# cvlab-kaist/CoPoNeRF

Hardware: AMD Instinct MI355X
Metric: rendered rays/sec (RealEstate10K-shaped 256x256 stereo pair, full-image render, 64 samples/ray) (higher is better)
Workload: dtype f16 (fp16-input/fp32-accumulate MFMA for the per-sample MLPs; f32 decoder; f64 geometry island); 1 GPU; configs[1]: 256x256 stereo pair (narrow rig), full-image render 65536 rays x 64 samples, 1 pair(s) per GPU, render path only (z/rel_pose/flow given, val=True); chunk_rays=65536, lanes=1, pairs_per_gpu=1

## Files before the change

### coponerf_amd/_hip.py

```python
from __future__ import annotations

import ctypes
import os
import re
from typing import Dict, List

_HERE = os.path.dirname(os.path.abspath(__file__))
LIB_PATH = os.environ.get("COPONERF_HIP_LIB") or os.path.join(_HERE, "libcoponerf_hip.so")
HEADER_PATH = os.path.join(os.path.dirname(_HERE), "include", "coponerf_hip.h")

_P, _I, _F = ctypes.c_void_p, ctypes.c_int, ctypes.c_float

SIGNATURES: Dict[str, List] = {
    "cpn_stream_create_cu_range": [_I, _I, ctypes.POINTER(ctypes.c_void_p)],
    "cpn_stream_destroy": [_P],
    "cpn_project_rays": [_P, _P, ctypes.c_longlong, _I, _I, _I, _P, _P, _P, _P],
    "cpn_sample_geometry": [_P, _P, _P, _P, _I, _I, _I, _I, _I, _I, _P, _P, _P, _P, _P, _P, _P],
    "cpn_nchw_to_nhwc_f16": [_P, _P, _I, _I, _I, _I, _P],
    "cpn_pack_weight_f16": [_P, _I, _I, _P, _I, _P],
    "cpn_pack_encode_weights": [_P, _I, _P, _P, _P],
    "cpn_node_features": [_P, _P, _P, _I, _I, _I, _P, _P],
    "cpn_encode_key": [_P, _P, _I, _I, _P, _P, _P, _P, _P, _P, _P, _I, _I, _I, _I, _I, _I, _P, _P, _I, _P],
    "cpn_local_units": [_I, _P, _P, _P, _I, _P, _P, _P, _I, _P, _P, _I, _P, _P, _I, _P, _P, _I, _I, _I, _I, _I, _I, _P, _P, _P, _P],
    "cpn_attend_units": [_I, _P, _P, _P, _I, _P, _P, _P, _I, _P, _P, _I, _P, _P, _I, _P, _P, _P, _I, _I, _I, _I, _I, _I, _P, _P, _P, _P, _P],
    "cpn_local_hidden": [_P, _P, _P, _I, _P, _P, _I, _I, _I, _I, _I, _I, _P, _P],
    "cpn_gemm_f16": [_P, _I, _P, _I, _P, _P, _I, _I, _I, _I, _I, _I, _P],
    "cpn_pack_gemm_frags": [_P, _I, _I, _I, _P, _P],
    "cpn_gemm_f16_fewrows": [_P, _I, _P, _P, _P, _I, _I, _I, _I, _I, _P],
    "cpn_attend_hidden": [_P, _P, _P, _P, _I, _I, _I, _I, _I, _I, _P, _P, _P],
    "cpn_node_features_f32": [_P, _P, _P, _I, _I, _I, _P, _P],
    "cpn_encode_hidden_f32": [_P, _P, _I, _I, _P, _P, _P, _P, _I, _I, _I, _I, _I, _I, _P, _P],
    "cpn_attend_hidden_f32": [_P, _P, _P, _I, _I, _I, _I, _I, _I, _P, _P, _P],
    "cpn_logit_guard": [_P, _I, _I, _I, _I, _I, _I, _P, _I, _P],
    "cpn_select_rays": [_P, _I, _F, _P, _P, _P],
    "cpn_encode_hidden_f32_rays": [_P, _P, _I, _I, _P, _P, _P, _P, _I, _I, _I, _I, _P, _I, _I, _P, _P],
    "cpn_attend_hidden_f32_rays": [_P, _P, _P, _I, _I, _I, _I, _P, _I, _I, _P, _P, _P],
    "cpn_linear_f32": [_P, _I, _P, _I, _P, _P, _I, _P, _I, _I, _I, _I, _I, _I, _P],
    "cpn_lightfield_decode": [_P, _P, _P, _P, _I, _I, _I, _P, _P, _P, _P],
    "cpn_ray_outputs": [_P, _P, _P, ctypes.c_longlong, _P, _P, _P, _I, _I, _I, _I, _P, _P, _P, _P, _P, _P, _P, _P],
    "cpn_attend_hidden_bwd": [_P, _P, _P, _P, _P, _P, _I, _I, _I, _I, _I, _I, _P, _P, _P, _P, _P],
    "cpn_attend_hidden_bwd_f32": [_P, _P, _P, _P, _P, _P, _I, _I, _I, _I, _I, _I, _P, _P, _P, _P],
    "cpn_hid_grad_combine": [_P, _P, _P, _P, _P, _P, _I, _I, _I, _I, _I, _I, _P, _P],
    "cpn_gemm_f16_combine": [_P, _I, _P, _I, _P, _P, _P, _P, _P, _I, _I, _I, _I, _I, _I, _I, _P, _P],
    "cpn_gemm_f16_combine_hs": [_P, _I, _P, _I, _P, _P, _P, _P, _P, _I, _I, _I, _I, _I, _I, _I, _P, _P],
    "cpn_gemm_f16_masked": [_P, _I, _P, _I, _P, _I, _P, _I, _I, _I, _I, _P],
    "cpn_wgrad_skinny_f16": [_P, _P, _I, ctypes.c_longlong, _P, _P, _P],
    "cpn_wgrad_tall_f16": [_P, _I, _P, _I, ctypes.c_longlong, _I, _I, _P, _P, _P, _P],
    "cpn_local_hidden_bwd": [_P, _P, _P, _P, _P, _I, _I, _I, _I, _P, _P, _P, _P],
    "cpn_gather_rows_bwd_level3": [_P, _I, _I, _I, _I, _P, _P, _I, _I, _I, _I, _I, _I, _P, _P, _P],
    "cpn_scatter_rows_tables": [_P, _I, _I, _I, _P, _P, _I, _I, _I, _I, _I, _I, _P, _P, _P],
    "cpn_node_features_bwd": [_P, _I, _I, _I, _P, _P, _P, _P],
    "cpn_scale_to_f16": [_P, ctypes.c_longlong, _F, _P, _P, _P, _P],
# ... 151 lines not shown
```

### coponerf_amd/csrc/attend_units.hip

```cpp
#include <algorithm>

#include "hid_sum.h"
#include "local_units_body.h"

namespace {

constexpr int HC = 1664;
constexpr int NCHUNK = HC / 8;
constexpr int NL = 4;
constexpr int NS = 2 * TG;
constexpr int AU_THREADS = (NL + NS) * 64;
constexpr int RU = HID_BLOCK_ROWS;
constexpr int LDS_MAX = 160 * 1024;

__device__ __forceinline__ float wave_max(float v) {
#pragma unroll
    for (int o = 32; o > 0; o >>= 1) v = fmaxf(v, __shfl_xor(v, o));
    return v;
}
__device__ __forceinline__ float wave_sum(float v) {
#pragma unroll
    for (int o = 32; o > 0; o >>= 1) v += __shfl_xor(v, o);
    return v;
}
// ... 76 lines not shown
        int b, r;
        size_t lray;
        const __half* hp;
    };
    auto ray_of = [&](unsigned k) {
        Ray o;
        const long long gq = geo.group0 + bid + (long long)k * nwg;
        o.b = (int)(gq / geo.groups_per_b);
        o.r = (int)(gq % geo.groups_per_b) * TG + j;
        const long long rayrel = (long long)o.b * R + o.r - geo.ray0;
        o.live = k < nmy && o.r < R && rayrel >= 0 && rayrel < geo.nrays;
        o.lray = (size_t)max(0LL, min(rayrel, (long long)geo.nrays - 1));
        o.hp = hid + o.lray * T * HC;
        return o;
    };
    auto issue = [&](const Ray& ray, half8 (&h0)[RU], half8 (&h1)[RU], int row) {
#pragma unroll
        for (int u = 0; u < RU; ++u) {
            const __half* rp = ray.hp + (size_t)(row + u) * HC;
            h0[u] = __builtin_nontemporal_load(reinterpret_cast<const half8*>(rp + off0));
            h1[u] = __builtin_nontemporal_load(reinterpret_cast<const half8*>(rp + off1));
        }
    };
    auto pin = [] {
        asm volatile("" ::: "memory");
        __builtin_amdgcn_sched_barrier(0);
    };
    half8 a0[RU], a1[RU], b0[RU], b1[RU];
    Ray nxt = ray_of(0);
    if (nxt.live && npair > 0) issue(nxt, a0, a1, 0);
    for (unsigned k = 0; k < nmy; ++k) {
        const Ray ray = nxt;
        nxt = ray_of(k + 1);
        const bool pre = nxt.live && npair > 0;
        const int b = ray.b, r = ray.r;
        group_barrier();
        if (!ray.live) {
            if (pre) issue(nxt, a0, a1, 0);
            continue;
        }

        const float* lg = ring + (k & 1) * (TG * T) + j * T;
        float* wt = wbuf + j * T;
        float lmax = -INFINITY;
        for (int row = lane; row < T; row += 64) lmax = fmaxf(lmax, lg[row] / 11.31f);
        const float gmax = wave_max(lmax);
        float ps[4] = {0.f, 0.f, 0.f, 0.f};
        for (int base = 0; base < T; base += 256) {
#pragma unroll
            for (int q = 0; q < 4; ++q) {
                const int row = base + q * 64 + lane;
                if (row < T) ps[q] += __expf(lg[row] / 11.31f - gmax);
            }
        }
#pragma unroll
        for (int q = 0; q < 4; ++q) ps[q] = wave_sum(ps[q]);
        const float inv = 1.0f / ((ps[0] + ps[1]) + (ps[2] + ps[3]));
        for (int row = lane; row < T; row += 64) {
            const float w = __expf(lg[row] / 11.31f - gmax) * inv;
            wt[row] = w;
            if (at_wt && half == 0) {
                const int v = row / S, s = row - v * S;
                at_wt[(((size_t)(b * V + v)) * R + r) * S + s] = w;
            }
        }
        asm volatile("s_waitcnt lgkmcnt(0)" ::: "memory");

        float acc0[8] = {0, 0, 0, 0, 0, 0, 0, 0}, acc1[8] = {0, 0, 0, 0, 0, 0, 0, 0};
        auto consume = [&](const half8 (&h0)[RU], const half8 (&h1)[RU], int row) {
#pragma unroll
            for (int u = 0; u < RU; ++u) {
                const float w = wt[row + u];
                hid_row_acc<true>(acc0, w, h0[u]);
                hid_row_acc<true>(acc1, w, h1[u]);
            }
        };
        if (npair > 0) {
            for (int p = 0; p + 1 < npair; ++p) {
                issue(ray, b0, b1, (2 * p + 1) * RU);
                pin();
                consume(a0, a1, 2 * p * RU);
                pin();
                issue(ray, a0, a1, (2 * p + 2) * RU);
                pin();
                consume(b0, b1, (2 * p + 1) * RU);
                pin();
            }
            issue(ray, b0, b1, (2 * npair - 1) * RU);
            pin();
            consume(a0, a1, (2 * npair - 2) * RU);
            pin();
            if (pre) issue(nxt, a0, a1, 0);
            pin();
            consume(b0, b1, (2 * npair - 1) * RU);
            pin();
        }
        for (int row = npair * 2 * RU; row < T; ++row) {
            const half8 h0 = __builtin_nontemporal_load(reinterpret_cast<const half8*>(ray.hp + (size_t)row * HC + off0));
            const half8 h1 = __builtin_nontemporal_load(reinterpret_cast<const half8*>(ray.hp + (size_t)row * HC + off1));
            const float w = wt[row];
            if (row < T - T % HID_BLOCK_ROWS) {
                hid_row_acc<true>(acc0, w, h0);
                hid_row_acc<true>(acc1, w, h1);
            } else {
                hid_row_acc<false>(acc0, w, h0);
                hid_row_acc<false>(acc1, w, h1);
            }
        }
        half8 o0, o1;
#pragma unroll
        for (int e = 0; e < 8; ++e) {
            o0[e] = (_Float16)acc0[e];
            o1[e] = (_Float16)acc1[e];
        }
        *reinterpret_cast<half8*>(hbar + ray.lray * HC + c0 * 8) = o0;
        if (live1) *reinterpret_cast<half8*>(hbar + ray.lray * HC + c1 * 8) = o1;
    }
}

template <int MODE>
int launch(const UnitArgs& args, const UnitGeo& geo, const __half* hid, __half* hbar, float* at_wt, float* logits, hipStream_t stream) {
    const int T = geo.V * geo.S;
    const size_t lds = unit_lds_bytes<MODE>() + (size_t)3 * TG * T * sizeof(float);
    CPN_REQUIRE(lds <= (size_t)LDS_MAX, CPN_E_SHAPE,
                "cpn_attend_units: V*S = %d needs %zu B of LDS (weights + 3 x 4 rays of logits / weights), the CU has %d", T, lds, LDS_MAX);
    auto kern = attend_units_kernel<MODE>;
    static bool attr_set = false;
    if (!attr_set) {
        hipError_t e = hipFuncSetAttribute((const void*)kern, hipFuncAttributeMaxDynamicSharedMemorySize, LDS_MAX);
        if (e != hipSuccess) {
            cpn_set_error("cpn_attend_units: cannot reserve %d B of LDS: %s", LDS_MAX, hipGetErrorString(e));
// ... 38 lines not shown
```

### coponerf_amd/csrc/gemm_f16.hip

```cpp
#include <algorithm>

#include "common.h"

namespace {

constexpr int BM = 256;
constexpr int BK = 64;
constexpr int ROW_BYTES = BK * 2;

typedef __attribute__((address_space(3))) void lds_void;
typedef const __attribute__((address_space(1))) void glb_void;

template <int NT>
struct Cfg {
    static constexpr int BN = NT * 16;
    static constexpr int UNITS_A = BM / 8;
    static constexpr int UNITS_B = BN / 8;
    static constexpr int UNITS = UNITS_A + UNITS_B;
    static constexpr int A_BYTES = BM * ROW_BYTES;
    static constexpr int B_BYTES = BN * ROW_BYTES;
    static constexpr int A_SLOTS = 3;
    static constexpr int B_SLOTS = 2;
    static constexpr int DUMP_BYTES = (UNITS_B % 8) ? 8 * 1024 : 0;
    static constexpr int LDS_BYTES = A_SLOTS * A_BYTES + B_SLOTS * B_BYTES + DUMP_BYTES;
// ... 7 lines not shown
    const int xcd = b & 7, idx = b >> 3;
    const int wg_x = (nwg >> 3) + (xcd < (nwg & 7) ? 1 : 0);
    const int q = total >> 3, r = total & 7;
    TileWalk t;
    t.begin = xcd < r ? xcd * (q + 1) : r * (q + 1) + (xcd - r) * q;
    t.end = t.begin + q + (xcd < r ? 1 : 0);
    t.step = wg_x;
    t.cur = t.begin + idx;
    return t;
}

struct CombineArgs {
    const float* w1; const float* dh1; const float* w2; const float* dh2;
    int V, R, S, ray0;
    int accum;
};
#ifndef CPN_HID_READ_NT
#define CPN_HID_READ_NT 1
#endif
template <int NT, bool OUT_F32, bool RELU, int DOT = 0>
__global__ __launch_bounds__(512) void gemm_f16_kernel(const __half* __restrict__ A, int lda,
                                                             const __half* __restrict__ W, int ldw,
                                                             const float* __restrict__ bias,
                                                             void* __restrict__ Cv, int ldc, int M, int K32, int n_tiles,
                                                             int total_tiles, const __half* __restrict__ Q = nullptr,
                                                             int ldq = 0, const __half* __restrict__ W2 = nullptr,
                                                             int ldw2 = 0, const float* __restrict__ bias2 = nullptr,
                                                             CombineArgs ca = CombineArgs{}) {
    using C_ = Cfg<NT>;
    constexpr int A_AUX = 0;
// ... 282 lines not shown
                    }
                }
                __builtin_amdgcn_fence(__ATOMIC_RELEASE, "wavefront");
            }
        } else {
#pragma unroll
            for (int nt = 0; nt < NT; ++nt) {
                const int n = n0 + nt * 16 + (lane >> 4) * 4;
                const f32x4 bv = *reinterpret_cast<const f32x4*>(bias + n);
#pragma unroll
                for (int mt = 0; mt < 2; ++mt) {
                    const int m = m0 + wave * 32 + mt * 16 + (lane & 15);
                    if (m >= M) continue;
                    f32x4 v = acc[mt][nt] + bv;
                    if (ca.accum) v += *reinterpret_cast<const f32x4*>((const float*)Cv + (size_t)m * ldc + n);
                    if (RELU) {
#pragma unroll
                        for (int i = 0; i < 4; ++i) v[i] = fmaxf(v[i], 0.0f);
                    }
                    *reinterpret_cast<f32x4*>((float*)Cv + (size_t)m * ldc + n) = v;
                }
            }
        }
    }
#undef CPN_INTERLEAVE_READS_MFMA
}

template <int NT, bool OUT_F32, bool RELU>
int launch(const __half* A, int lda, const __half* W, int ldw, const float* bias, void* C, int ldc, int M, int N,
           int K32, hipStream_t stream, int accum = 0) {
    using C_ = Cfg<NT>;
    const size_t lds = C_::LDS_BYTES;
    auto kern = gemm_f16_kernel<NT, OUT_F32, RELU>;
    static bool attr_set = false;
    if (!attr_set) {
        hipError_t e = hipFuncSetAttribute((const void*)kern, hipFuncAttributeMaxDynamicSharedMemorySize, (int)lds);
        if (e != hipSuccess) {
            cpn_set_error("cpn_gemm_f16: cannot reserve %zu B of LDS: %s", lds, hipGetErrorString(e));
            return (int)e;
        }
        attr_set = true;
    }
    const int n_tiles = N / C_::BN;
    const long long total = (long long)cpn_cdiv(M, BM) * n_tiles;
    if (total >= (1LL << 31)) {
        cpn_set_error("cpn_gemm_f16: %lld output tiles exceed the 32-bit tile index", total);
        return CPN_E_SHAPE;
    }
    const int num_cu = cpn_stream_cus((void*)stream);
    dim3 grid((unsigned)std::min<long long>(total, num_cu));
    hipLaunchKernelGGL(kern, grid, dim3(512), lds, stream, A, lda, W, ldw, bias, C, ldc, M, K32, n_tiles, (int)total,
                       (const __half*)nullptr, 0, (const __half*)nullptr, 0, (const float*)nullptr,
                       CombineArgs{nullptr, nullptr, nullptr, nullptr, 0, 0, 0, 0, accum});
    CPN_LAUNCH_CHECK("cpn_gemm_f16");
    return 0;
}

template <int NT>
int launch_combine(const __half* A, int lda, const __half* W, int ldw, const __half* hid, int ldh, const CombineArgs& ca,
                   __half* out, int ld, int M, int N, int K32, hipStream_t stream) {
    using C_ = Cfg<NT>;
    const size_t lds = C_::LDS_BYTES;
    auto kern = gemm_f16_kernel<NT, false, false, 3>;
    static bool attr_set = false;
    if (!attr_set) {
        hipError_t e = hipFuncSetAttribute((const void*)kern, hipFuncAttributeMaxDynamicSharedMemorySize, (int)lds);
        if (e != hipSuccess) {
            cpn_set_error("cpn_gemm_f16_combine: cannot reserve %zu B of LDS: %s", lds, hipGetErrorString(e));
// ... 36 lines not shown
    out[i] = *reinterpret_cast<const half8*>(W + (size_t)(t * 16 + (lane & 15)) * ldw + ks * 32 + (lane >> 4) * 8);
}

#ifndef CPN_FEW_NT
#define CPN_FEW_NT 4
#endif
#ifndef CPN_FEW_DEPTH
#define CPN_FEW_DEPTH 4
#endif
#ifndef CPN_FEW_RT
#define CPN_FEW_RT 2
#endif
constexpr int FEW_NT = CPN_FEW_NT, FEW_RT = CPN_FEW_RT;
__global__ __launch_bounds__(256) void gemm_f16_fewrows_kernel(const __half* __restrict__ A, int lda,
                                                               const half8* __restrict__ Wp, const float* __restrict__ bias,
                                                               float* __restrict__ C, int ldc, int M, int N, int K32, int relu) {
    constexpr int NT = FEW_NT, RT = FEW_RT, D = CPN_FEW_DEPTH;
    const int lane = threadIdx.x & 63, wave = threadIdx.x >> 6;
    const int r = lane & 15, g = lane >> 4;
    const int m0 = blockIdx.x * 16 * RT;
    const int ntiles = N >> 4;
    const int tile0 = (blockIdx.y * 4 + wave) * NT;
    if (tile0 >= ntiles) return;
    const int rl = lane >> 2, pl = lane & 3;
    const int to_frag = (4 * r + g) * 4;
    const __half* ap[RT];
#pragma unroll
    for (int q = 0; q < RT; ++q) {
        const int row = m0 + q * 16 + rl < M ? m0 + q * 16 + rl : M - 1;
        ap[q] = A + (size_t)row * lda + pl * 8;
    }
// ... 68 lines not shown
        for (int q = 0; q < RT; ++q) xl[q] = frag(xl[q]);
#pragma unroll
        for (int t = 0; t < NT; ++t)
#pragma unroll
            for (int q = 0; q < RT; ++q) acc[q][t] = __builtin_amdgcn_mfma_f32_16x16x32_f16(wl[t], xl[q], acc[q][t], 0, 0, 0);
    }
#pragma unroll
    for (int q = 0; q < RT; ++q) {
        const int m = m0 + q * 16 + r;
        if (m >= M) continue;
#pragma unroll
        for (int t = 0; t < NT; ++t) {
            if (tile0 + t >= ntiles) continue;
            const int n = (tile0 + t) * 16 + g * 4;
            f32x4 v = acc[q][t] + *reinterpret_cast<const f32x4*>(bias + n);
            if (relu) {
#pragma unroll
                for (int i = 0; i < 4; ++i) v[i] = fmaxf(v[i], 0.0f);
            }
            *reinterpret_cast<f32x4*>(C + (size_t)m * ldc + n) = v;
        }
    }
}

}

extern "C" int cpn_pack_gemm_frags(const uint16_t* W, int ldw, int N, int K, uint16_t* out, void* stream) {
    CPN_REQUIRE(W && out, CPN_E_ARG, "cpn_pack_gemm_frags: null pointer");
    CPN_REQUIRE(N > 0 && (N % 16) == 0 && K > 0 && (K % 32) == 0 && ldw >= K && (ldw % 8) == 0, CPN_E_SHAPE,
                "cpn_pack_gemm_frags: need N %% 16 == 0, K %% 32 == 0, ldw >= K (got N=%d K=%d ldw=%d)", N, K, ldw);
// ... 3 lines not shown
                       K / 32, (half8*)out);
    CPN_LAUNCH_CHECK("cpn_pack_gemm_frags");
    return 0;
}

extern "C" int cpn_gemm_f16_fewrows(const uint16_t* A, int lda, const uint16_t* Wp, const float* bias, float* C, int ldc, int M,
                                    int N, int K, int relu, void* stream) {
    CPN_REQUIRE(A && Wp && bias && C, CPN_E_ARG, "cpn_gemm_f16_fewrows: null pointer");
    CPN_REQUIRE(M > 0 && N > 0 && (N % 16) == 0 && K > 0 && (K % 32) == 0, CPN_E_SHAPE,
                "cpn_gemm_f16_fewrows: need N %% 16 == 0 and K %% 32 == 0 (got N=%d K=%d)", N, K);
    CPN_REQUIRE(lda >= K && (lda % 8) == 0 && ldc >= N && (ldc % 4) == 0, CPN_E_SHAPE, "cpn_gemm_f16_fewrows: bad leading dimension");
    CPN_REQUIRE(((uintptr_t)A % 16) == 0 && ((uintptr_t)Wp % 16) == 0 && ((uintptr_t)C % 16) == 0 && ((uintptr_t)bias % 16) == 0,
                CPN_E_ARG, "cpn_gemm_f16_fewrows: pointers must be 16-byte aligned");
    dim3 grid(cpn_cdiv(M, 16 * FEW_RT), cpn_cdiv(N / 16, 4 * FEW_NT));
    hipLaunchKernelGGL(gemm_f16_fewrows_kernel, grid, dim3(256), 0, (hipStream_t)stream, (const __half*)A, lda, (const half8*)Wp, bias,
                       C, ldc, M, N, K / 32, relu);
    CPN_LAUNCH_CHECK("cpn_gemm_f16_fewrows");
    return 0;
}

extern "C" int cpn_gemm_f16(const uint16_t* A, int lda, const uint16_t* W, int ldw, const float* bias, void* C,
                            int ldc, int M, int N, int K, int relu, int out_f32, void* stream) {
    CPN_REQUIRE(A && W && bias && C, CPN_E_ARG, "cpn_gemm_f16: null pointer");
    CPN_REQUIRE(M > 0 && N > 0 && K > 0 && (K % 32) == 0, CPN_E_SHAPE, "cpn_gemm_f16: K=%d must be a multiple of 32", K);
    CPN_REQUIRE(lda >= K && ldw >= K && (lda % 8) == 0 && (ldw % 8) == 0, CPN_E_SHAPE,
                "cpn_gemm_f16: lda=%d / ldw=%d must be >= K=%d and multiples of 8 halves", lda, ldw, K);
    CPN_REQUIRE((long long)256 * lda * 2 < (1LL << 31) && (long long)N * ldw * 2 < (1LL << 31), CPN_E_SHAPE,
                "cpn_gemm_f16: tile exceeds the 32-bit buffer offset range");
    CPN_REQUIRE(ldc >= N && (ldc % 8) == 0, CPN_E_SHAPE, "cpn_gemm_f16: ldc=%d must be >= N and a multiple of 8", ldc);
    CPN_REQUIRE(((uintptr_t)A % 16) == 0 && ((uintptr_t)W % 16) == 0 && ((uintptr_t)C % 16) == 0 &&
                    ((uintptr_t)bias % 16) == 0, CPN_E_ARG, "cpn_gemm_f16: pointers must be 16-byte aligned");
    const hipStream_t s = (hipStream_t)stream;
    const __half* a = (const __half*)A;
    const __half* w = (const __half*)W;
    if (N % 208 == 0) return dispatch<13>(a, lda, w, ldw, bias, C, ldc, M, N, K / 32, relu, out_f32, s);
    if (N % 128 == 0) return dispatch<8>(a, lda, w, ldw, bias, C, ldc, M, N, K / 32, relu, out_f32, s);
    cpn_set_error("cpn_gemm_f16: N=%d is neither a multiple of 208 nor of 128", N);
    return CPN_E_SHAPE;
}

namespace {

template <int LDH>
int gemm_f16_combine(const char* name, const uint16_t* dkh, int lda, const uint16_t* Wt, int ldw, const uint16_t* hid,
                     const float* w1, const float* dh1, const float* w2, const float* dh2, int B, int V, int R, int S, int ray0,
                     int nrays, int K, uint16_t* out, void* stream) {
    CPN_REQUIRE(dkh && Wt && hid && out && (!w1 || dh1) && (!w2 || dh2), CPN_E_ARG, "%s: null pointer", name);
    CPN_REQUIRE(B > 0 && V == 2 && R > 0 && S > 0 && (S % 16) == 0, CPN_E_SHAPE, "%s: need V == 2, S %% 16 == 0", name);
    CPN_REQUIRE(ray0 >= 0 && nrays > 0 && (long long)ray0 + nrays <= (long long)B * R, CPN_E_SHAPE,
                "%s: ray range outside B*R", name);
    CPN_REQUIRE(K > 0 && (K % 32) == 0 && lda >= K && ldw >= K && (lda % 8) == 0 && (ldw % 8) == 0, CPN_E_SHAPE,
                "%s: bad K / leading dimension", name);
// ... 49 lines not shown
```

### coponerf_amd/csrc/linear_f32.hip

```cpp
#include "common.h"

namespace {

#ifndef CPN_LIN_DEPTH
#define CPN_LIN_DEPTH 2
#endif
template <int NT>
__global__ __launch_bounds__(256) void linear_f32_kernel(const float* __restrict__ X, int ldx,
                                                         const float* __restrict__ W, int ldw,
                                                         const float* __restrict__ bias,
                                                         const float* __restrict__ res, int ldr,
                                                         float* __restrict__ Y, int ldy, int M, int N, int K,
                                                         int relu_in, int relu_out) {
    constexpr int D = CPN_LIN_DEPTH;
    const int lane = threadIdx.x & 63, wave = threadIdx.x >> 6;
    const int m0 = (blockIdx.x * 4 + wave) * 16;
    const int t0 = blockIdx.y * NT;
    if (m0 >= M) return;
    const int fi = lane & 15, fg = lane >> 4;
    int xr = m0 + fi;
    xr = xr < M ? xr : M - 1;
    const float* xp = X + (size_t)xr * ldx + fg * 4;
    f32x4 acc[NT];
#pragma unroll
// ... 57 lines not shown
            continue;
        }
#pragma unroll
        for (int i = 0; i < 4; ++i) {
            const int n = n0 + i;
            if (n >= N) continue;
            float v = acc[t][i];
            if (bias) v += bias[n];
            if (res) v += res[(size_t)m * ldr + n];
            if (relu_out) v = fmaxf(v, 0.0f);
            Y[(size_t)m * ldy + n] = v;
        }
    }
}

}

extern "C" int cpn_linear_f32(const float* X, int ldx, const float* W, int ldw, const float* bias, const float* res,
                              int ldr, float* Y, int ldy, int M, int N, int K, int relu_in, int relu_out,
                              void* stream) {
    CPN_REQUIRE(X && W && Y, CPN_E_ARG, "cpn_linear_f32: null pointer");
    CPN_REQUIRE(M > 0 && N > 0 && N <= 128 && K > 0 && (K % 16) == 0, CPN_E_SHAPE,
                "cpn_linear_f32: need N<=128 and K%%16==0 (got N=%d K=%d)", N, K);
    CPN_REQUIRE(ldx >= K && ldw >= K && (ldx % 4) == 0 && (ldw % 4) == 0 && ldy >= N && (!res || ldr >= N),
                CPN_E_SHAPE, "cpn_linear_f32: bad leading dimensions");
    CPN_REQUIRE(((uintptr_t)X % 16) == 0 && ((uintptr_t)W % 16) == 0, CPN_E_ARG, "cpn_linear_f32: X/W must be 16-B aligned");
    const hipStream_t s = (hipStream_t)stream;
    dim3 grid(cpn_cdiv(M, 64)), block(256);
    const int ntiles = (int)cpn_cdiv(N, 16);
    if (N <= 16)
// ... 13 lines not shown
```

### coponerf_amd/render.py

```python
from __future__ import annotations

import ctypes
import math
import os
from typing import Dict, List, Optional, Sequence, Tuple

import torch

from . import _hip, render_f32
from ._hip import call

V = 2


def _ptr(t: Optional[torch.Tensor]) -> int:
    return 0 if t is None else t.data_ptr()


def _stream() -> int:
    return _hip.stream_handle()


def _flat_on_device(mats: Sequence[Optional[torch.Tensor]]) -> Optional[torch.Tensor]:
    live = [m for m in mats if m is not None]
# ... 271 lines not shown
            return func(*args, **kwargs)


class RenderEngine:

    GEMM_WEIGHTS = {
        "key_map_2": (128, 128, 128),
        "query_embed_2": (128, 128, 128),
        "query_repeat_embed_2": (128, 128, 128),
    }

    WORKSPACE_SHARE = 0.25
    FREE_SHARE = 0.5
    MAX_AUTO_CHUNK = 65536
    ATTEND_UNITS_MAX_T = 1684
    FEW_ROWS = 4096
    AUTO_THRESHOLD = 0.5062
    PRECISIONS = ("f16", "f32", "auto")
    TRAIN_PRECISIONS = ("f16", "f32")
    SETTINGS = ("chunk_rays", "lanes", "grad_scale_target", "call_lanes", "lazy_pixel_val", "precision", "f32_chunk_rays",
                "auto_threshold", "train_precision")

    def __init__(self, chunk_rays: int = 0, lanes: int = 1):
        self.chunk_rays = int(chunk_rays) or int(os.environ.get("COPONERF_CHUNK_RAYS", "0"))
        self.grad_scale_target = 256.0
        self.lanes = max(1, int(lanes))
        self._lane_streams: List[torch.cuda.Stream] = []
        self.precision = os.environ.get("COPONERF_PRECISION", "f16")
        self.f32_chunk_rays = 16384
        self.auto_threshold = self.AUTO_THRESHOLD
# ... 550 lines not shown
        score = self._buf("guard.score", (nray_total,), f32, dev) if auto else None
        C = min(self.chunk_rays if self.chunk_rays > 0 else self._auto_chunk(S, dev, nray_total), nray_total)
        T = V * S
        fused = T <= self.ATTEND_UNITS_MAX_T
        nchunks = (nray_total + C - 1) // C
        nlanes = min(self.lanes, nchunks)
        if nlanes > 1 and (len(self._lane_streams) < nlanes or self._lane_streams[0].device != dev):
            self._lane_streams = [torch.cuda.Stream(device=dev) for _ in range(nlanes)]
        main = torch.cuda.current_stream()

        def lane_buffers(lane):
            t = lambda name, shape, dt: self._buf(f"{name}.{lane}", shape, dt, dev)
            rows128 = ((C + 3) // 4 + B + 1) * V * ((S + 3) // 4) * 16
            return {"lg": t("lg", (C * T,), f32) if (auto or not fused) else None,
                    "z1": t("z1", (C, 416), f32), "ze": t("ze", (C, 128), f32), "addq": t("addq", (C, 128), f32),
                    "hbar": t("hbar", (C, 1664), f16), "zs": t("zs", (C, 416), f32),
                    "hid": t("hid", (C * T * 2, 832), f16), "khf": t("khf", (rows128, 128), f16)}

        def timed(name, flops, fn):
            prof = self.profile
            if prof is None:
                return fn()
            e0, e1 = torch.cuda.Event(enable_timing=True), torch.cuda.Event(enable_timing=True)
            e0.record()
            fn()
            e1.record()
            prof.setdefault(name, []).append((e0, e1, flops))

        def value_fold(s, hbar, out, m):
            if m <= self.FEW_ROWS:
                fn = lambda: call("cpn_gemm_f16_fewrows", hbar.data_ptr(), 1664, w["value_fold.wpk"].data_ptr(),
                                  w["value_fold.b"].data_ptr(), out.data_ptr(), 416, m, 416, 1664, 0, s)
            else:
                fn = lambda: call("cpn_gemm_f16", hbar.data_ptr(), 1664, w["value_fold.w16"].data_ptr(), 1664,
                                  w["value_fold.b"].data_ptr(), out.data_ptr(), 416, m, 416, 1664, 0, 1, s)
            timed("gemm_f16:value_fold", 2.0 * m * 416 * 1664, fn)

        def run_chunk(ray0, bf, s):
            n = min(C, nray_total - ray0)
            rows2 = n * T * 2
            timed("encode_key", 2.0 * rows2 * 832 * 835, lambda: call(
                "cpn_encode_key", tabs[0].data_ptr(), maps[3].data_ptr(), H, W, pixel_val.data_ptr(), sec_grid.data_ptr(),
                pe6.data_ptr(), w["enc.frag"].data_ptr(), w["query_encode_latent.b"].data_ptr(), w["key_fold.wpk"].data_ptr(),
                w["key_fold.b"].data_ptr(), B, V, R, S, ray0, n, bf["hid"].data_ptr(), bf["khf"].data_ptr(), 1, s))
            lg = bf["lg"].data_ptr() if (auto or not fused) else 0
            r1 = (0, loc8.data_ptr(), coords9.data_ptr(), w["query_embed.w"].data_ptr(), 16,
                  w["query_embed.b"].data_ptr(), 0, w["query_embed_2.w16"].data_ptr(), 128, w["query_embed_2.b"].data_ptr(),
                  w["key_map_2.w16"].data_ptr(), 128, w["key_map_2.b"].data_ptr(), 0, 0, 0, bf["khf"].data_ptr())
            if fused:
                timed("attend_units:round1", 2.0 * n * T * (128 * (128 + 128 + 16) + 1664), lambda: call(
                    "cpn_attend_units", *r1, bf["hid"].data_ptr(), B, V, R, S, ray0, n, lvu.data_ptr(),
                    bf["hbar"].data_ptr(), at_wt.data_ptr(), lg, s))
            else:
                timed("local_units:query_embed+key_map_2", 2.0 * n * T * 128 * (128 + 128 + 16), lambda: call(
                    "cpn_local_units", *r1, B, V, R, S, ray0, n, 0, lvu.data_ptr(), lg, s))
                timed("attend_hidden:round1", 2.0 * n * T * 1664, lambda: call(
                    "cpn_attend_hidden", 0, 0, lg, bf["hid"].data_ptr(), B, V, R, S, ray0, n,
                    bf["hbar"].data_ptr(), at_wt.data_ptr(), s))
            if auto:
                timed("logit_guard:round1", 0.0, lambda: call(
                    "cpn_logit_guard", lg, B, V, R, S, ray0, n, score.data_ptr(), 0, s))
            z1, ze, addq = bf["z1"], bf["ze"], bf["addq"]
            value_fold(s, bf["hbar"], z1, n)
            call("cpn_linear_f32", z1.data_ptr(), 416, w["encode_latent.w"].data_ptr(), 416,
                 w["encode_latent.b"].data_ptr(), 0, 0, ze.data_ptr(), 128, n, 128, 416, 0, 0, s)
            call("cpn_linear_f32", ze.data_ptr(), 128, w["query_repeat_embed.w_z"].data_ptr(), 128, 0, 0, 0,
                 addq.data_ptr(), 128, n, 128, 128, 0, 0, s)
            r2 = (2, loc8.data_ptr(), coords9.data_ptr(), w["query_repeat_embed.w_l"].data_ptr(), 16,
                  w["query_repeat_embed.b"].data_ptr(), addq.data_ptr(), w["query_repeat_embed_2.w16"].data_ptr(), 128,
                  w["query_repeat_embed_2.b"].data_ptr(), w["query_embed_2.w16"].data_ptr(), 128, w["query_embed_2.b"].data_ptr(),
                  w["query_embed.w"].data_ptr(), 16, w["query_embed.b"].data_ptr(), 0)
            if fused:
                timed("attend_units:round2", 2.0 * n * T * (128 * (2 * 128 + 2 * 16) + 1664), lambda: call(
                    "cpn_attend_units", *r2, bf["hid"].data_ptr(), B, V, R, S, ray0, n, lvu.data_ptr(),
                    bf["hbar"].data_ptr(), 0, lg, s))
            else:
                timed("local_units:round2+query_embed", 2.0 * n * T * 128 * (2 * 128 + 2 * 16), lambda: call(
                    "cpn_local_units", *r2, B, V, R, S, ray0, n, 0, lvu.data_ptr(), lg, s))
                timed("attend_hidden:round2", 2.0 * n * T * 1664, lambda: call(
                    "cpn_attend_hidden", 0, 0, lg, bf["hid"].data_ptr(), B, V, R, S, ray0, n,
                    bf["hbar"].data_ptr(), 0, s))
            if auto:
                timed("logit_guard:round2", 0.0, lambda: call(
                    "cpn_logit_guard", lg, B, V, R, S, ray0, n, score.data_ptr(), 1, s))
            value_fold(s, bf["hbar"], bf["zs"], n)
            torch.add(bf["zs"][:n], z1[:n], alpha=float(V), out=zl[ray0:ray0 + n])

        dims = (B, R, S, H, W)
        f32_inputs = lambda: self._f32_inputs(pre[8], w, H, W)
        if self.precision == "f32":
            render_f32.per_sample(*f32_inputs(), g, zl, at_wt, dims, self.f32_chunk_rays, self._buf, s)
        elif nlanes == 1:
            bf = lane_buffers(0)
            for ray0 in range(0, nray_total, C):
                run_chunk(ray0, bf, s)
        else:
            ready = torch.cuda.Event()
            ready.record()
            for ci, ray0 in enumerate(range(0, nray_total, C)):
                lane = ci % nlanes
                st = self._lane_streams[lane]
# ... 43 lines not shown
```

### include/coponerf_hip.h

```cpp
#ifndef COPONERF_HIP_H
#define COPONERF_HIP_H

#include <stdint.h>

#ifdef __cplusplus
extern "C" {
#endif

#define CPN_ABI_VERSION 12

#define CPN_E_ARG   (-1)
#define CPN_E_SHAPE (-2)

#define CPN_CAM_STRIDE 96
#define CPN_CAM_TQ    0
#define CPN_CAM_M     16
#define CPN_CAM_AOWN  32
#define CPN_CAM_AOTH  48
#define CPN_CAM_KQ    64
#define CPN_CAM_KC    68
#define CPN_CAM_KO    72
#define CPN_CAM_KN    76


// ... 28 lines not shown
int cpn_encode_key(const uint16_t* tab, const uint16_t* map3, int H, int W, const float* pixel_val,
                   const float* sec_grid, const float* pe6, const uint16_t* wfrag, const float* bias,
                   const uint16_t* kwring, const float* kbias, int B, int V, int R, int S, int ray0, int nrays,
                   uint16_t* hid, uint16_t* kh, int kh_units, void* stream);
long long cpn_encode_units(int B, int R, int S, int ray0, int nrays);
int cpn_local_units(int mode, const float* loc8, const float* coords9, const float* w1, int ldw1, const float* b1,
                    const float* add, const uint16_t* w2, int ldw2, const float* b2, const uint16_t* wk2, int ldwk2,
                    const float* bk2, const float* w1b, int ldw1b, const float* b1b, const uint16_t* kh_u, int B, int V,
                    int R, int S, int ray0, int nrays, uint16_t* ce_u, const float* lv_u, float* logits, void* stream);

int cpn_gemm_f16(const uint16_t* A, int lda, const uint16_t* W, int ldw, const float* bias,
                 void* C, int ldc, int M, int N, int K, int relu, int out_f32, void* stream);
int cpn_pack_gemm_frags(const uint16_t* W, int ldw, int N, int K, uint16_t* out, void* stream);
int cpn_gemm_f16_fewrows(const uint16_t* A, int lda, const uint16_t* Wp, const float* bias, float* C, int ldc, int M, int N,
                         int K, int relu, void* stream);

int cpn_attend_hidden(const uint16_t* qa, const uint16_t* qb, const float* logits, const uint16_t* hid, int B, int V,
                      int R, int S, int ray0, int nrays, uint16_t* hbar, float* at_wt, void* stream);

int cpn_attend_units(int mode, const float* loc8, const float* coords9, const float* w1, int ldw1, const float* b1,
                     const float* add, const uint16_t* w2, int ldw2, const float* b2, const uint16_t* wk2, int ldwk2,
                     const float* bk2, const float* w1b, int ldw1b, const float* b1b, const uint16_t* kh_u, const uint16_t* hid,
                     int B, int V, int R, int S, int ray0, int nrays, const float* lv_u, uint16_t* hbar, float* at_wt,
                     float* logits, void* stream);

int cpn_linear_f32(const float* X, int ldx, const float* W, int ldw, const float* bias, const float* res, int ldr,
                   float* Y, int ldy, int M, int N, int K, int relu_in, int relu_out, void* stream);

#define CPN_LIGHTFIELD_PACK_FLOATS (128 * 32 + 128 + 3 * (128 * 416 + 128 + 2 * (128 * 128 + 128)) + 16 * 128 + 16)
int cpn_lightfield_decode(const float* coords9, const float* z_local, const float* wpack, const uint8_t* overlaps,
                          int B, int V, int R, float* rgb, float* valid, float* rgb_raw, void* stream);

#define CPN_RAYC_STRIDE 64
int cpn_ray_outputs(const float* at_wt, const float* pt, const float* uv, long long uv_batch_stride, const float* rayc,
                    const uint8_t* mask2, const float* flow_up, int B, int V, int R, int S, long long* at_wt_max,
                    float* depth_ray, float* t_to_c1, float* t_to_c2, uint8_t* mask_c2, uint8_t* match_mask,
                    float* c2_to_c1, void* stream);


int cpn_node_features_f32(const float* map0, const float* map1, const float* map2, int H, int W, int nimg, float* feat,
                          void* stream);

// ... 180 lines not shown
```

Before: 2.936 million rays/s.

## Fuse residual add into value_fold GEMM and chain two f32 linears

```diff
diff --git a/coponerf_amd/_hip.py b/coponerf_amd/_hip.py
--- a/coponerf_amd/_hip.py
+++ b/coponerf_amd/_hip.py
@@ -27,6 +27,8 @@
     "cpn_gemm_f16": [_P, _I, _P, _I, _P, _P, _I, _I, _I, _I, _I, _I, _P],
     "cpn_pack_gemm_frags": [_P, _I, _I, _I, _P, _P],
     "cpn_gemm_f16_fewrows": [_P, _I, _P, _P, _P, _I, _I, _I, _I, _I, _P],
+    "cpn_gemm_f16_res": [_P, _I, _P, _I, _P, _P, _I, _F, _P, _I, _I, _I, _I, _P],
+    "cpn_gemm_f16_fewrows_res": [_P, _I, _P, _P, _P, _I, _F, _P, _I, _I, _I, _I, _P],
     "cpn_attend_hidden": [_P, _P, _P, _P, _I, _I, _I, _I, _I, _I, _P, _P, _P],
     "cpn_node_features_f32": [_P, _P, _P, _I, _I, _I, _P, _P],
     "cpn_encode_hidden_f32": [_P, _P, _I, _I, _P, _P, _P, _P, _I, _I, _I, _I, _I, _I, _P, _P],
@@ -36,6 +38,7 @@
     "cpn_encode_hidden_f32_rays": [_P, _P, _I, _I, _P, _P, _P, _P, _I, _I, _I, _I, _P, _I, _I, _P, _P],
     "cpn_attend_hidden_f32_rays": [_P, _P, _P, _I, _I, _I, _I, _P, _I, _I, _P, _P, _P],
     "cpn_linear_f32": [_P, _I, _P, _I, _P, _P, _I, _P, _I, _I, _I, _I, _I, _I, _P],
+    "cpn_linear2_f32": [_P, _I, _P, _I, _P, _P, _I, _P, _P, _I, _P, _I, _I, _I, _P],
     "cpn_lightfield_decode": [_P, _P, _P, _P, _I, _I, _I, _P, _P, _P, _P],
     "cpn_ray_outputs": [_P, _P, _P, ctypes.c_longlong, _P, _P, _P, _I, _I, _I, _I, _P, _P, _P, _P, _P, _P, _P, _P],
     "cpn_attend_hidden_bwd": [_P, _P, _P, _P, _P, _P, _I, _I, _I, _I, _I, _I, _P, _P, _P, _P, _P],
diff --git a/coponerf_amd/csrc/attend_units.hip b/coponerf_amd/csrc/attend_units.hip
--- a/coponerf_amd/csrc/attend_units.hip
+++ b/coponerf_amd/csrc/attend_units.hip
@@ -114,12 +114,15 @@
         o.hp = hid + o.lray * T * HC;
         return o;
     };
+    auto load_row = [&](const Ray& ray, unsigned voff, int row) {
+        const __amdgpu_buffer_rsrc_t rs = __builtin_amdgcn_make_buffer_rsrc((void*)ray.hp, 0, T * HC * 2, 0x00020000);
+        return __builtin_bit_cast(half8, __builtin_amdgcn_raw_buffer_load_b128(rs, (int)voff * 2, row * HC * 2, 2));
+    };
     auto issue = [&](const Ray& ray, half8 (&h0)[RU], half8 (&h1)[RU], int row) {
 #pragma unroll
         for (int u = 0; u < RU; ++u) {
-            const __half* rp = ray.hp + (size_t)(row + u) * HC;
-            h0[u] = __builtin_nontemporal_load(reinterpret_cast<const half8*>(rp + off0));
-            h1[u] = __builtin_nontemporal_load(reinterpret_cast<const half8*>(rp + off1));
+            h0[u] = load_row(ray, off0, row + u);
+            h1[u] = load_row(ray, off1, row + u);
         }
     };
     auto pin = [] {
@@ -128,17 +131,12 @@
     };
     half8 a0[RU], a1[RU], b0[RU], b1[RU];
     Ray nxt = ray_of(0);
-    if (nxt.live && npair > 0) issue(nxt, a0, a1, 0);
+    if (npair > 0) issue(nxt, a0, a1, 0);
     for (unsigned k = 0; k < nmy; ++k) {
         const Ray ray = nxt;
         nxt = ray_of(k + 1);
-        const bool pre = nxt.live && npair > 0;
         const int b = ray.b, r = ray.r;
         group_barrier();
-        if (!ray.live) {
-            if (pre) issue(nxt, a0, a1, 0);
-            continue;
-        }
 
         const float* lg = ring + (k & 1) * (TG * T) + j * T;
         float* wt = wbuf + j * T;
@@ -159,7 +157,7 @@
         for (int row = lane; row < T; row += 64) {
             const float w = __expf(lg[row] / 11.31f - gmax) * inv;
             wt[row] = w;
-            if (at_wt && half == 0) {
+            if (at_wt && half == 0 && ray.live) {
                 const int v = row / S, s = row - v * S;
                 at_wt[(((size_t)(b * V + v)) * R + r) * S + s] = w;
             }
@@ -174,30 +172,35 @@
                 hid_row_acc<true>(acc0, w, h0[u]);
                 hid_row_acc<true>(acc1, w, h1[u]);
             }
+        };
+        auto done = [&] {
+            asm volatile("" : "+v"(acc0[0]), "+v"(acc0[1]), "+v"(acc0[2]), "+v"(acc0[3]), "+v"(acc0[4]), "+v"(acc0[5]), "+v"(acc0[6]),
+                         "+v"(acc0[7]), "+v"(acc1[0]), "+v"(acc1[1]), "+v"(acc1[2]), "+v"(acc1[3]), "+v"(acc1[4]), "+v"(acc1[5]),
+                         "+v"(acc1[6]), "+v"(acc1[7])::"memory");
+            __builtin_amdgcn_sched_barrier(0);
         };
         if (npair > 0) {
             for (int p = 0; p + 1 < npair; ++p) {
                 issue(ray, b0, b1, (2 * p + 1) * RU);
                 pin();
                 consume(a0, a1, 2 * p * RU);
-                pin();
+                done();
                 issue(ray, a0, a1, (2 * p + 2) * RU);
                 pin();
                 consume(b0, b1, (2 * p + 1) * RU);
-                pin();
+                done();
             }
             issue(ray, b0, b1, (2 * npair - 1) * RU);
             pin();
             consume(a0, a1, (2 * npair - 2) * RU);
-            pin();
-            if (pre) issue(nxt, a0, a1, 0);
+            done();
+            issue(nxt, a0, a1, 0);
             pin();
             consume(b0, b1, (2 * npair - 1) * RU);
-            pin();
+            done();
         }
         for (int row = npair * 2 * RU; row < T; ++row) {
-            const half8 h0 = __builtin_nontemporal_load(reinterpret_cast<const half8*>(ray.hp + (size_t)row * HC + off0));
-            const half8 h1 = __builtin_nontemporal_load(reinterpret_cast<const half8*>(ray.hp + (size_t)row * HC + off1));
+            const half8 h0 = load_row(ray, off0, row), h1 = load_row(ray, off1, row);
             const float w = wt[row];
             if (row < T - T % HID_BLOCK_ROWS) {
                 hid_row_acc<true>(acc0, w, h0);
@@ -213,8 +216,8 @@
             o0[e] = (_Float16)acc0[e];
             o1[e] = (_Float16)acc1[e];
         }
-        *reinterpret_cast<half8*>(hbar + ray.lray * HC + c0 * 8) = o0;
-        if (live1) *reinterpret_cast<half8*>(hbar + ray.lray * HC + c1 * 8) = o1;
+        if (ray.live) *reinterpret_cast<half8*>(hbar + ray.lray * HC + c0 * 8) = o0;
+        if (ray.live && live1) *reinterpret_cast<half8*>(hbar + ray.lray * HC + c1 * 8) = o1;
     }
 }
 
diff --git a/coponerf_amd/csrc/gemm_f16.hip b/coponerf_amd/csrc/gemm_f16.hip
--- a/coponerf_amd/csrc/gemm_f16.hip
+++ b/coponerf_amd/csrc/gemm_f16.hip
@@ -45,6 +45,7 @@
     const float* w1; const float* dh1; const float* w2; const float* dh2;
     int V, R, S, ray0;
     int accum;
+    const float* res; int ldr; float alpha;
 };
 #ifndef CPN_HID_READ_NT
 #define CPN_HID_READ_NT 1
@@ -357,6 +358,11 @@
                     if (m >= M) continue;
                     f32x4 v = acc[mt][nt] + bv;
                     if (ca.accum) v += *reinterpret_cast<const f32x4*>((const float*)Cv + (size_t)m * ldc + n);
+                    if (ca.res) {
+                        const f32x4 z = *reinterpret_cast<const f32x4*>(ca.res + (size_t)m * ca.ldr + n);
+#pragma unroll
+                        for (int i = 0; i < 4; ++i) v[i] = __builtin_fmaf(ca.alpha, z[i], v[i]);
+                    }
                     if (RELU) {
 #pragma unroll
                         for (int i = 0; i < 4; ++i) v[i] = fmaxf(v[i], 0.0f);
@@ -371,7 +377,7 @@
 
 template <int NT, bool OUT_F32, bool RELU>
 int launch(const __half* A, int lda, const __half* W, int ldw, const float* bias, void* C, int ldc, int M, int N,
-           int K32, hipStream_t stream, int accum = 0) {
+           int K32, hipStream_t stream, int accum = 0, const float* res = nullptr, int ldr = 0, float alpha = 0.0f) {
     using C_ = Cfg<NT>;
     const size_t lds = C_::LDS_BYTES;
     auto kern = gemm_f16_kernel<NT, OUT_F32, RELU>;
@@ -394,7 +400,7 @@
     dim3 grid((unsigned)std::min<long long>(total, num_cu));
     hipLaunchKernelGGL(kern, grid, dim3(512), lds, stream, A, lda, W, ldw, bias, C, ldc, M, K32, n_tiles, (int)total,
                        (const __half*)nullptr, 0, (const __half*)nullptr, 0, (const float*)nullptr,
-                       CombineArgs{nullptr, nullptr, nullptr, nullptr, 0, 0, 0, 0, accum});
+                       CombineArgs{nullptr, nullptr, nullptr, nullptr, 0, 0, 0, 0, accum, res, ldr, alpha});
     CPN_LAUNCH_CHECK("cpn_gemm_f16");
     return 0;
 }
@@ -461,7 +467,8 @@
 constexpr int FEW_NT = CPN_FEW_NT, FEW_RT = CPN_FEW_RT;
 __global__ __launch_bounds__(256) void gemm_f16_fewrows_kernel(const __half* __restrict__ A, int lda,
                                                                const half8* __restrict__ Wp, const float* __restrict__ bias,
-                                                               float* __restrict__ C, int ldc, int M, int N, int K32, int relu) {
+                                                               float* __restrict__ C, int ldc, int M, int N, int K32, int relu,
+                                                               const float* __restrict__ res, int ldr, float alpha) {
     constexpr int NT = FEW_NT, RT = FEW_RT, D = CPN_FEW_DEPTH;
     const int lane = threadIdx.x & 63, wave = threadIdx.x >> 6;
     const int r = lane & 15, g = lane >> 4;
@@ -560,6 +567,11 @@
             if (tile0 + t >= ntiles) continue;
             const int n = (tile0 + t) * 16 + g * 4;
             f32x4 v = acc[q][t] + *reinterpret_cast<const f32x4*>(bias + n);
+            if (res) {
+                const f32x4 z = *reinterpret_cast<const f32x4*>(res + (size_t)m * ldr + n);
+#pragma unroll
+                for (int i = 0; i < 4; ++i) v[i] = __builtin_fmaf(alpha, z[i], v[i]);
+            }
             if (relu) {
 #pragma unroll
                 for (int i = 0; i < 4; ++i) v[i] = fmaxf(v[i], 0.0f);
@@ -593,8 +605,24 @@
                 CPN_E_ARG, "cpn_gemm_f16_fewrows: pointers must be 16-byte aligned");
     dim3 grid(cpn_cdiv(M, 16 * FEW_RT), cpn_cdiv(N / 16, 4 * FEW_NT));
     hipLaunchKernelGGL(gemm_f16_fewrows_kernel, grid, dim3(256), 0, (hipStream_t)stream, (const __half*)A, lda, (const half8*)Wp, bias,
-                       C, ldc, M, N, K / 32, relu);
+                       C, ldc, M, N, K / 32, relu, (const float*)nullptr, 0, 0.0f);
     CPN_LAUNCH_CHECK("cpn_gemm_f16_fewrows");
+    return 0;
+}
+
+extern "C" int cpn_gemm_f16_fewrows_res(const uint16_t* A, int lda, const uint16_t* Wp, const float* bias, const float* res, int ldr,
+                                        float alpha, float* C, int ldc, int M, int N, int K, void* stream) {
+    CPN_REQUIRE(A && Wp && bias && res && C, CPN_E_ARG, "cpn_gemm_f16_fewrows_res: null pointer");
+    CPN_REQUIRE(M > 0 && N > 0 && (N % 16) == 0 && K > 0 && (K % 32) == 0, CPN_E_SHAPE,
+                "cpn_gemm_f16_fewrows_res: need N %% 16 == 0 and K %% 32 == 0 (got N=%d K=%d)", N, K);
+    CPN_REQUIRE(lda >= K && (lda % 8) == 0 && ldc >= N && (ldc % 4) == 0 && ldr >= N && (ldr % 4) == 0, CPN_E_SHAPE,
+                "cpn_gemm_f16_fewrows_res: bad leading dimension");
+    CPN_REQUIRE(((uintptr_t)A % 16) == 0 && ((uintptr_t)Wp % 16) == 0 && ((uintptr_t)C % 16) == 0 && ((uintptr_t)bias % 16) == 0 &&
+                    ((uintptr_t)res % 16) == 0, CPN_E_ARG, "cpn_gemm_f16_fewrows_res: pointers must be 16-byte aligned");
+    dim3 grid(cpn_cdiv(M, 16 * FEW_RT), cpn_cdiv(N / 16, 4 * FEW_NT));
+    hipLaunchKernelGGL(gemm_f16_fewrows_kernel, grid, dim3(256), 0, (hipStream_t)stream, (const __half*)A, lda, (const half8*)Wp, bias,
+                       C, ldc, M, N, K / 32, 0, res, ldr, alpha);
+    CPN_LAUNCH_CHECK("cpn_gemm_f16_fewrows_res");
     return 0;
 }
 
@@ -615,6 +643,27 @@
     if (N % 208 == 0) return dispatch<13>(a, lda, w, ldw, bias, C, ldc, M, N, K / 32, relu, out_f32, s);
     if (N % 128 == 0) return dispatch<8>(a, lda, w, ldw, bias, C, ldc, M, N, K / 32, relu, out_f32, s);
     cpn_set_error("cpn_gemm_f16: N=%d is neither a multiple of 208 nor of 128", N);
+    return CPN_E_SHAPE;
+}
+
+extern "C" int cpn_gemm_f16_res(const uint16_t* A, int lda, const uint16_t* W, int ldw, const float* bias, const float* res, int ldr,
+                                float alpha, float* C, int ldc, int M, int N, int K, void* stream) {
+    CPN_REQUIRE(A && W && bias && res && C, CPN_E_ARG, "cpn_gemm_f16_res: null pointer");
+    CPN_REQUIRE(M > 0 && N > 0 && K > 0 && (K % 32) == 0, CPN_E_SHAPE, "cpn_gemm_f16_res: K=%d must be a multiple of 32", K);
+    CPN_REQUIRE(lda >= K && ldw >= K && (lda % 8) == 0 && (ldw % 8) == 0, CPN_E_SHAPE,
+                "cpn_gemm_f16_res: lda=%d / ldw=%d must be >= K=%d and multiples of 8 halves", lda, ldw, K);
+    CPN_REQUIRE((long long)256 * lda * 2 < (1LL << 31) && (long long)N * ldw * 2 < (1LL << 31), CPN_E_SHAPE,
+                "cpn_gemm_f16_res: tile exceeds the 32-bit buffer offset range");
+    CPN_REQUIRE(ldc >= N && (ldc % 8) == 0 && ldr >= N && (ldr % 4) == 0, CPN_E_SHAPE,
+                "cpn_gemm_f16_res: ldc=%d must be >= N and a multiple of 8, ldr=%d >= N and a multiple of 4", ldc, ldr);
+    CPN_REQUIRE(((uintptr_t)A % 16) == 0 && ((uintptr_t)W % 16) == 0 && ((uintptr_t)C % 16) == 0 && ((uintptr_t)bias % 16) == 0 &&
+                    ((uintptr_t)res % 16) == 0, CPN_E_ARG, "cpn_gemm_f16_res: pointers must be 16-byte aligned");
+    const hipStream_t s = (hipStream_t)stream;
+    const __half* a = (const __half*)A;
+    const __half* w = (const __half*)W;
+    if (N % 208 == 0) return launch<13, true, false>(a, lda, w, ldw, bias, C, ldc, M, N, K / 32, s, 0, res, ldr, alpha);
+    if (N % 128 == 0) return launch<8, true, false>(a, lda, w, ldw, bias, C, ldc, M, N, K / 32, s, 0, res, ldr, alpha);
+    cpn_set_error("cpn_gemm_f16_res: N=%d is neither a multiple of 208 nor of 128", N);
     return CPN_E_SHAPE;
 }
 
diff --git a/coponerf_amd/csrc/linear_f32.hip b/coponerf_amd/csrc/linear_f32.hip
--- a/coponerf_amd/csrc/linear_f32.hip
+++ b/coponerf_amd/csrc/linear_f32.hip
@@ -95,6 +95,99 @@
     }
 }
 
+__global__ __launch_bounds__(256) void linear2_f32_kernel(const float* __restrict__ X, int ldx, const float* __restrict__ W1, int ldw1,
+                                                          const float* __restrict__ b1, const float* __restrict__ W2, int ldw2,
+                                                          const float* __restrict__ b2, float* __restrict__ Y1, int ldy1,
+                                                          float* __restrict__ Y2, int ldy2, int M, int K) {
+    constexpr int D = CPN_LIN_DEPTH, NT = 8;
+    const int lane = threadIdx.x & 63, wave = threadIdx.x >> 6;
+    const int m0 = (blockIdx.x * 4 + wave) * 16;
+    if (m0 >= M) return;
+    const int fi = lane & 15, fg = lane >> 4;
+    int xr = m0 + fi;
+    xr = xr < M ? xr : M - 1;
+    const float* xp = X + (size_t)xr * ldx + fg * 4;
+    const int m = m0 + fi;
+
+    auto product = [&](const float* __restrict__ W, int ldw, int nkb, auto&& xfrag, f32x4 (&acc)[NT]) {
+        const float* wp[NT];
+#pragma unroll
+        for (int t = 0; t < NT; ++t) {
+            acc[t] = f32x4{0.f, 0.f, 0.f, 0.f};
+            wp[t] = W + (size_t)(t * 16 + fi) * ldw + fg * 4;
+        }
+        f32x4 xa[D], wa[D][NT];
+        auto fetch = [&](int d, int kb) {
+            xa[d] = xfrag(kb);
+#pragma unroll
+            for (int t = 0; t < NT; ++t) wa[d][t] = *reinterpret_cast<const f32x4*>(wp[t] + kb * 16);
+        };
+#pragma unroll
+        for (int d = 0; d < D; ++d)
+            if (d < nkb) fetch(d, d);
+        for (int kb0 = 0; kb0 < nkb; kb0 += D) {
+#pragma unroll
+            for (int d = 0; d < D; ++d) {
+                const int kb = kb0 + d;
+                if (kb < nkb) {
+                    const f32x4 xv = xa[d];
+#pragma unroll
+                    for (int t = 0; t < NT; ++t)
+#pragma unroll
+                        for (int e = 0; e < 4; ++e)
+                            acc[t] = __builtin_amdgcn_mfma_f32_16x16x4f32(wa[d][t][e], xv[e], acc[t], 0, 0, 0);
+                    if (kb + D < nkb) fetch(d, kb + D);
+                }
+            }
+        }
+    };
+    auto finish = [&](f32x4 (&acc)[NT], const float* __restrict__ bias, float* __restrict__ Y, int ldy) {
+        const bool vec = (ldy & 3) == 0 && (((uintptr_t)Y | (uintptr_t)bias) & 15) == 0;
+#pragma unroll
+        for (int t = 0; t < NT; ++t) {
+            const int n0 = t * 16 + fg * 4;
+            if (bias) {
+                if (vec) acc[t] += *reinterpret_cast<const f32x4*>(bias + n0);
+                else {
+#pragma unroll
+                    for (int i = 0; i < 4; ++i) acc[t][i] += bias[n0 + i];
+                }
+            }
+            if (!Y || m >= M) continue;
+            if (vec) *reinterpret_cast<f32x4*>(Y + (size_t)m * ldy + n0) = acc[t];
+            else {
+#pragma unroll
+                for (int i = 0; i < 4; ++i) Y[(size_t)m * ldy + n0 + i] = acc[t][i];
+            }
+        }
+    };
+    f32x4 mid[NT], acc[NT];
+    product(W1, ldw1, K >> 4, [&](int kb) { return *reinterpret_cast<const f32x4*>(xp + kb * 16); }, mid);
+    finish(mid, b1, Y1, ldy1);
+    auto mid_frag = [&](int kb) {
+        f32x4 v = mid[0];
+#pragma unroll
+        for (int t = 1; t < NT; ++t) v = kb == t ? mid[t] : v;
+        return v;
+    };
+    product(W2, ldw2, NT, mid_frag, acc);
+    finish(acc, b2, Y2, ldy2);
+}
+
+}
+
+extern "C" int cpn_linear2_f32(const float* X, int ldx, const float* W1, int ldw1, const float* b1, const float* W2, int ldw2,
+                               const float* b2, float* Y1, int ldy1, float* Y2, int ldy2, int M, int K, void* stream) {
+    CPN_REQUIRE(X && W1 && W2 && Y2, CPN_E_ARG, "cpn_linear2_f32: null pointer");
+    CPN_REQUIRE(M > 0 && K > 0 && (K % 16) == 0, CPN_E_SHAPE, "cpn_linear2_f32: need K%%16==0 (got K=%d)", K);
+    CPN_REQUIRE(ldx >= K && ldw1 >= K && ldw2 >= 128 && (ldx % 4) == 0 && (ldw1 % 4) == 0 && (ldw2 % 4) == 0 && ldy2 >= 128 &&
+                    (!Y1 || ldy1 >= 128), CPN_E_SHAPE, "cpn_linear2_f32: bad leading dimensions");
+    CPN_REQUIRE(((uintptr_t)X % 16) == 0 && ((uintptr_t)W1 % 16) == 0 && ((uintptr_t)W2 % 16) == 0, CPN_E_ARG,
+                "cpn_linear2_f32: X/W1/W2 must be 16-B aligned");
+    hipLaunchKernelGGL(linear2_f32_kernel, dim3(cpn_cdiv(M, 64)), dim3(256), 0, (hipStream_t)stream, X, ldx, W1, ldw1, b1, W2, ldw2,
+                       b2, Y1, ldy1, Y2, ldy2, M, K);
+    CPN_LAUNCH_CHECK("cpn_linear2_f32");
+    return 0;
 }
 
 extern "C" int cpn_linear_f32(const float* X, int ldx, const float* W, int ldw, const float* bias, const float* res,
diff --git a/coponerf_amd/render.py b/coponerf_amd/render.py
--- a/coponerf_amd/render.py
+++ b/coponerf_amd/render.py
@@ -309,6 +309,7 @@
     FREE_SHARE = 0.5
     MAX_AUTO_CHUNK = 65536
     ATTEND_UNITS_MAX_T = 1684
+    LINEAR2_MIN_ROWS = 16384
     FEW_ROWS = 4096
     AUTO_THRESHOLD = 0.5062
     PRECISIONS = ("f16", "f32", "auto")
@@ -889,7 +890,7 @@
             rows128 = ((C + 3) // 4 + B + 1) * V * ((S + 3) // 4) * 16
             return {"lg": t("lg", (C * T,), f32) if (auto or not fused) else None,
                     "z1": t("z1", (C, 416), f32), "ze": t("ze", (C, 128), f32), "addq": t("addq", (C, 128), f32),
-                    "hbar": t("hbar", (C, 1664), f16), "zs": t("zs", (C, 416), f32),
+                    "hbar": t("hbar", (C, 1664), f16),
                     "hid": t("hid", (C * T * 2, 832), f16), "khf": t("khf", (rows128, 128), f16)}
 
         def timed(name, flops, fn):
@@ -902,13 +903,20 @@
             e1.record()
             prof.setdefault(name, []).append((e0, e1, flops))
 
-        def value_fold(s, hbar, out, m):
-            if m <= self.FEW_ROWS:
+        def value_fold(s, hbar, out, m, res=None):
+            few = m <= self.FEW_ROWS
+            if few and res is None:
                 fn = lambda: call("cpn_gemm_f16_fewrows", hbar.data_ptr(), 1664, w["value_fold.wpk"].data_ptr(),
                                   w["value_fold.b"].data_ptr(), out.data_ptr(), 416, m, 416, 1664, 0, s)
-            else:
+            elif few:
+                fn = lambda: call("cpn_gemm_f16_fewrows_res", hbar.data_ptr(), 1664, w["value_fold.wpk"].data_ptr(),
+                                  w["value_fold.b"].data_ptr(), res.data_ptr(), 416, float(V), out.data_ptr(), 416, m, 416, 1664, s)
+            elif res is None:
                 fn = lambda: call("cpn_gemm_f16", hbar.data_ptr(), 1664, w["value_fold.w16"].data_ptr(), 1664,
                                   w["value_fold.b"].data_ptr(), out.data_ptr(), 416, m, 416, 1664, 0, 1, s)
+            else:
+                fn = lambda: call("cpn_gemm_f16_res", hbar.data_ptr(), 1664, w["value_fold.w16"].data_ptr(), 1664,
+                                  w["value_fold.b"].data_ptr(), res.data_ptr(), 416, float(V), out.data_ptr(), 416, m, 416, 1664, s)
             timed("gemm_f16:value_fold", 2.0 * m * 416 * 1664, fn)
 
         def run_chunk(ray0, bf, s):
@@ -937,10 +945,14 @@
                     "cpn_logit_guard", lg, B, V, R, S, ray0, n, score.data_ptr(), 0, s))
             z1, ze, addq = bf["z1"], bf["ze"], bf["addq"]
             value_fold(s, bf["hbar"], z1, n)
-            call("cpn_linear_f32", z1.data_ptr(), 416, w["encode_latent.w"].data_ptr(), 416,
-                 w["encode_latent.b"].data_ptr(), 0, 0, ze.data_ptr(), 128, n, 128, 416, 0, 0, s)
-            call("cpn_linear_f32", ze.data_ptr(), 128, w["query_repeat_embed.w_z"].data_ptr(), 128, 0, 0, 0,
-                 addq.data_ptr(), 128, n, 128, 128, 0, 0, s)
+            if n > self.LINEAR2_MIN_ROWS:
+                call("cpn_linear2_f32", z1.data_ptr(), 416, w["encode_latent.w"].data_ptr(), 416, w["encode_latent.b"].data_ptr(),
+                     w["query_repeat_embed.w_z"].data_ptr(), 128, 0, 0, 0, addq.data_ptr(), 128, n, 416, s)
+            else:
+                call("cpn_linear_f32", z1.data_ptr(), 416, w["encode_latent.w"].data_ptr(), 416,
+                     w["encode_latent.b"].data_ptr(), 0, 0, ze.data_ptr(), 128, n, 128, 416, 0, 0, s)
+                call("cpn_linear_f32", ze.data_ptr(), 128, w["query_repeat_embed.w_z"].data_ptr(), 128, 0, 0, 0,
+                     addq.data_ptr(), 128, n, 128, 128, 0, 0, s)
             r2 = (2, loc8.data_ptr(), coords9.data_ptr(), w["query_repeat_embed.w_l"].data_ptr(), 16,
                   w["query_repeat_embed.b"].data_ptr(), addq.data_ptr(), w["query_repeat_embed_2.w16"].data_ptr(), 128,
                   w["query_repeat_embed_2.b"].data_ptr(), w["query_embed_2.w16"].data_ptr(), 128, w["query_embed_2.b"].data_ptr(),
@@ -958,8 +970,7 @@
             if auto:
                 timed("logit_guard:round2", 0.0, lambda: call(
                     "cpn_logit_guard", lg, B, V, R, S, ray0, n, score.data_ptr(), 1, s))
-            value_fold(s, bf["hbar"], bf["zs"], n)
-            torch.add(bf["zs"][:n], z1[:n], alpha=float(V), out=zl[ray0:ray0 + n])
+            value_fold(s, bf["hbar"], zl[ray0:ray0 + n], n, res=z1)
 
         dims = (B, R, S, H, W)
         f32_inputs = lambda: self._f32_inputs(pre[8], w, H, W)
diff --git a/include/coponerf_hip.h b/include/coponerf_hip.h
--- a/include/coponerf_hip.h
+++ b/include/coponerf_hip.h
@@ -66,6 +66,10 @@
 int cpn_pack_gemm_frags(const uint16_t* W, int ldw, int N, int K, uint16_t* out, void* stream);
 int cpn_gemm_f16_fewrows(const uint16_t* A, int lda, const uint16_t* Wp, const float* bias, float* C, int ldc, int M, int N,
                          int K, int relu, void* stream);
+int cpn_gemm_f16_res(const uint16_t* A, int lda, const uint16_t* W, int ldw, const float* bias, const float* res, int ldr,
+                     float alpha, float* C, int ldc, int M, int N, int K, void* stream);
+int cpn_gemm_f16_fewrows_res(const uint16_t* A, int lda, const uint16_t* Wp, const float* bias, const float* res, int ldr,
+                             float alpha, float* C, int ldc, int M, int N, int K, void* stream);
 
 int cpn_attend_hidden(const uint16_t* qa, const uint16_t* qb, const float* logits, const uint16_t* hid, int B, int V,
                       int R, int S, int ray0, int nrays, uint16_t* hbar, float* at_wt, void* stream);
@@ -78,6 +82,8 @@
 
 int cpn_linear_f32(const float* X, int ldx, const float* W, int ldw, const float* bias, const float* res, int ldr,
                    float* Y, int ldy, int M, int N, int K, int relu_in, int relu_out, void* stream);
+int cpn_linear2_f32(const float* X, int ldx, const float* W1, int ldw1, const float* b1, const float* W2, int ldw2,
+                    const float* b2, float* Y1, int ldy1, float* Y2, int ldy2, int M, int K, void* stream);
 
 #define CPN_LIGHTFIELD_PACK_FLOATS (128 * 32 + 128 + 3 * (128 * 416 + 128 + 2 * (128 * 128 + 128)) + 16 * 128 + 16)
 int cpn_lightfield_decode(const float* coords9, const float* z_local, const float* wpack, const uint8_t* overlaps,
```

Result: slower. 2.879 million rays/s (-1.9%).
